# Aikku93/ulc-codec

Hardware: AMD Instinct MI355X
Metric: encode+decode Msamples/s at BlockSize=2048 stereo (channel-samples through encode+decode, VBR -50, 32 blocks per stream per call) (higher is better)
Workload: dtype f32; 1 GPU; vbr50 (configs[1] encode, configs[2] decode): Batch=4096 independent 44.1 kHz stereo streams/GPU x 32 blocks, BlockSize=2048, VBR -50; step = encode then decode; config=vbr50, mode=both, streams_per_gpu=4096, block_size=2048, channels=2, parallelism=batch split over 1 GPU(s), no collective on the data path

## Files before the change

### ulc-codec_amd/csrc/ulcx_enc.hip

```cpp
#include "ulcx_enc_dev.h"

static size_t ulcx_enc_xf_lds_bytes(int BS, int C) {
    if (BS > 8192) return (size_t)BS * 4;
    int ps = ulcx_xf_pad_shift(BS, C);
    size_t z = (size_t)4 * (BS + (BS >> ps)) * 4;
    size_t full = z + (size_t)BS * 2 + 32 + (C > 2 ? (size_t)BS * 2 : 0);
    return full <= ULCX_LDS_LIMIT ? full : z + (size_t)BS * 2 + 32;
}

static size_t ulcx_enc_xfa_lds_bytes(int BS, int C) {
    if (BS > 8192) return (size_t)BS * 4;
    int ps = ulcx_xf_pad_shift(BS, C);
    return (size_t)2 * (BS + (BS >> ps)) * 4 + (size_t)BS * 2 + 32;
}

#define CK(x) do { hipError_t e_ = (x); if (e_ != hipSuccess) { ulcx_set_error("%s: %s", #x, hipGetErrorString(e_)); return ULCX_ERR_HIP; } } while (0)
#define TRY(x) do { int rc_ = (x); if (rc_) return rc_; } while (0)

typedef void (*RangeKernel)(UlcxEncCtx, int, int);
typedef void (*PassKernel)(UlcxEncCtx, int);
typedef void (*CallKernel)(UlcxEncCtx);

static RangeKernel wc_energy_fn(const UlcxEncCtx &c) { return c.pcm16 ? k_wc_energy<int16_t> : k_wc_energy<float>; }
static RangeKernel wc_ef_fn(const UlcxEncCtx &c) { return c.pcm16 ? k_wc_ef<EF_NW, int16_t> : k_wc_ef<EF_NW, float>; }
static CallKernel state_update_fn(const UlcxEncCtx &c) { return c.pcm16 ? k_state_update<int16_t> : k_state_update<float>; }

template <typename IN> static RangeKernel xf_fn_in(const UlcxEncCtx &c, bool mdctOnly) {
    if (c.BS > 8192) return mdctOnly ? k_xfa_big<IN> : k_xf_big<IN>;
    if (c.C == 2) return mdctOnly ? k_xfa<true, IN> : k_xf<true, IN>;
    return mdctOnly ? k_xfa<false, IN> : k_xf<false, IN>;
}
static RangeKernel xf_fn(const UlcxEncCtx &c, bool mdctOnly) { return c.pcm16 ? xf_fn_in<int16_t>(c, mdctOnly) : xf_fn_in<float>(c, mdctOnly); }

template <int PASS> static PassKernel select_fn_pass(const UlcxEncCtx &c, bool pair, bool rates) {
#define SEL(R, L) (rates ? (PassKernel)k_select_wave_rates<R, L, PASS> : (PassKernel)k_select_wave<R, L, PASS>)
    switch (c.C * c.BS / 64) {
        case 128:
            if (pair) return rates ? k_select_pair_rates<64, 12, PASS> : k_select_pair<64, 12, PASS>;
            return SEL(128, 0);
        case 64: return c.lgBS == 11 ? SEL(64, 11) : SEL(64, 0);
        case 32: return SEL(32, 0);
        case 16: return SEL(16, 0);
        case 8:  return SEL(8, 0);
        case 4:  return SEL(4, 0);
        default: return nullptr;
    }
#undef SEL
}
static PassKernel select_fn(const UlcxEncCtx &c, bool pair, bool rates, int pass) {
    return pass == 1 ? select_fn_pass<1>(c, pair, rates) : pass == 2 ? select_fn_pass<2>(c, pair, rates) : select_fn_pass<0>(c, pair, rates);
}

static int allow_lds(const void *fn, size_t lds) {
    if (lds > 48 * 1024) CK(hipFuncSetAttribute(fn, hipFuncAttributeMaxDynamicSharedMemorySize, (int)lds));
    return ULCX_OK;
}

static void launch_wc_energy(const UlcxEncCtx &c, unsigned grid, hipStream_t st, int k0, int k1) {
    hipLaunchKernelGGL(wc_energy_fn(c), dim3(grid), dim3(WG), 0, st, c, k0, k1);
}

static void launch_wc_ef(const UlcxEncCtx &c, hipStream_t st, int k0, int k1) {
    static_assert(EF_LDS_BYTES <= 48 * 1024, "k_wc_ef: raise the dynamic LDS limit with hipFuncSetAttribute");
    hipLaunchKernelGGL(wc_ef_fn(c), dim3((c.B + EF_SPW - 1) / EF_SPW), dim3(EF_NW * 64), EF_LDS_BYTES, st, c, k0, k1);
}

static void launch_state_update(const UlcxEncCtx &c, hipStream_t st) {
    hipLaunchKernelGGL(state_update_fn(c), dim3(c.B), dim3(WG), 0, st, c);
}

const char *const ulcx_enc_stage_names[ULCX_ENC_STAGES_REPORTED] = {
    "k_wc_energy", "k_wc_forward", "k_wc_backward", "k_wc_integrate", "k_wc_decide",
    "k_xf", "k_cplx", "k_pbark", "k_mask",
    "k_select", "k_nbark", "(k_nline: gone)", "k_heapsel", "k_nsums", "k_tails", "k_encode_wave", "k_encode_units", "k_pack", "cbr_probe_passes", "k_state_update", "wc_pipeline_exposed",
};

struct StageMarks { hipEvent_t *ev; int stage; };
#define MARK(mk, s) do { if ((mk).ev) CK(hipEventRecord((mk).ev[(mk).stage++], s)); } while (0)

enum { ULCX_FRONT_ENCODE = 0, ULCX_FRONT_ANALYSE = 1, ULCX_FRONT_ANALYSE_KXF = 2, ULCX_FRONT_WC_ONLY = 3 };
static int launch_front(const UlcxEncCtx &c, hipStream_t st, StageMarks &mk, const UlcxEncAux &aux, const int what) {
    UlcxEncSync &sy = aux.sync;
    hipStream_t side = sy.side, side2 = sy.side2, side3 = sy.side3;
    const int SG = (c.B + 63) / 64;
    const int nCh = aux.wcPipe;
    const bool mdctOnly = (what == ULCX_FRONT_ANALYSE);
    const RangeKernel xf = (what == ULCX_FRONT_WC_ONLY) ? nullptr : xf_fn(c, mdctOnly);
    const size_t lds = mdctOnly ? ulcx_enc_xfa_lds_bytes(c.BS, c.C) : ulcx_enc_xf_lds_bytes(c.BS, c.C);
    if (xf) TRY(allow_lds((const void *)xf, lds));
    auto transform = [&](int k0, int k1) {
        if (xf) hipLaunchKernelGGL(xf, dim3((unsigned)((c.B * (k1 - k0) + 7) / 8) * 8), dim3(WG), lds, st, c, k0, k1);
    };
    const bool wcFuse = c.C == 2 && aux.wcFuse;
    aux.nXf = 0;
    if (nCh <= 1) {
        if (wcFuse) { MARK(mk, st); launch_wc_ef(c, st, 0, c.K);                                                  MARK(mk, st); }
        else {
        launch_wc_energy(c, (unsigned)(SG * ((c.K * c.BS) / 64)), st, 0, c.K);                                    MARK(mk, st);
        hipLaunchKernelGGL(k_wc_forward, dim3((c.B * 2 + 63) / 64), dim3(64), 0, st, c, 0, c.K);                  MARK(mk, st);
        }
        hipLaunchKernelGGL(k_wc_backward, dim3(SG * c.K), dim3(64), 0, st, c, 0, c.K);                            MARK(mk, st);
        hipLaunchKernelGGL(k_wc_integrate, dim3((c.B + 63) / 64), dim3(64), 0, st, c, 0, c.K);                    MARK(mk, st);
        hipLaunchKernelGGL(k_wc_decide, dim3((c.B * c.K + 63) / 64), dim3(64), 0, st, c, 0, c.K);                 MARK(mk, st);
        transform(0, c.K);
        MARK(mk, st);
        return ULCX_OK;
    }
    for (int i = 0; i < 5; i++) MARK(mk, st);
    const UlcxFrontPlan fp = ulcx_front_plan(c.K, nCh, aux.wcSteps);
    const int nW = fp.nW;
    const int *cut = fp.cut, *wcs = fp.wcs;
    CK(hipEventRecord(sy.wcStart, st));
    CK(hipStreamWaitEvent(side, sy.wcStart, 0));
    int jx = 0;
    for (int w = 0; w < nW; w++) {
        const int k0 = wcs[w], k1 = wcs[w + 1], kc = k1 - k0;
        if (wcFuse) launch_wc_ef(c, side, k0, k1);
        else {
            launch_wc_energy(c, (unsigned)(SG * ((kc * c.BS) / 64)), side, k0, k1);
            hipLaunchKernelGGL(k_wc_forward, dim3((c.B * 2 + 63) / 64), dim3(64), 0, side, c, k0, k1);
        }
        CK(hipEventRecord(sy.wcForward[w], side));
        CK(hipStreamWaitEvent(side2, sy.wcForward[w], 0));
        hipLaunchKernelGGL(k_wc_backward, dim3(SG * kc), dim3(64), 0, side2, c, k0, k1);
        CK(hipEventRecord(sy.wcBackward[w], side2));
        CK(hipStreamWaitEvent(side3, sy.wcBackward[w], 0));
        hipLaunchKernelGGL(k_wc_integrate, dim3((c.B + 63) / 64), dim3(64), 0, side3, c, k0, k1);
        hipLaunchKernelGGL(k_wc_decide, dim3((c.B * kc + 63) / 64), dim3(64), 0, side3, c, k0, k1);
        CK(hipEventRecord(sy.wcDecided[w], side3));
        while (jx < nCh && cut[jx + 1] <= k1) {
            CK(hipStreamWaitEvent(st, sy.wcDecided[w], 0));
            if (mk.ev) CK(hipEventRecord(sy.xfTiming[2 * jx], st));
            if (!(ULCX_DBG(c) & 0x2000))
            transform(cut[jx], cut[jx + 1]);
            if (mk.ev) CK(hipEventRecord(sy.xfTiming[2 * jx + 1], st));
            CK(hipEventRecord(sy.xfChunkDone[jx], st));
            jx++;
        }
    }
    aux.nXf = nCh;
    MARK(mk, st);
    for (int j = 0; j < nCh; j++) {
        CK(hipStreamWaitEvent(side, sy.xfChunkDone[j], 0));
        const int kc2 = cut[j + 1] - cut[j];
        if (what == ULCX_FRONT_ENCODE) hipLaunchKernelGGL(k_cplx, dim3((c.B * kc2 + 63) / 64), dim3(64), 0, side, c, cut[j], cut[j + 1]);
        else hipLaunchKernelGGL(k_cplxa, dim3((c.B * kc2 + 63) / 64), dim3(64), 0, side, c, cut[j], cut[j + 1]);
    }
    CK(hipEventRecord(sy.cplxChunksDone, side));
    return ULCX_OK;
}

struct EncPlan {
    int NB, N, nUnits;
    bool aside;
    int probes;
    size_t barkLds;
    bool selWave, selPair;
    size_t selLds;
    int ldsEntries, fbGrid; size_t heapLds;
    WaveCaps capS, capM, capF;
    bool haveFull, haveMid;
    int nsSlots;
};
static int enc_probes(const UlcxEncCtx &c, int N) {
    int n = 0;
    if (c.mode != ULCX_MODE_VBR || c.rates != nullptr) { n = 2; for (int m = N; m > 1; m >>= 1) n++; }
    return n;
}
static EncPlan enc_plan(const UlcxEncCtx &c, const UlcxEncAux &aux) {
    EncPlan p;
    p.NB = c.B * c.K; p.N = c.C * c.BS; p.nUnits = p.NB * c.C * 4;
    p.aside = aux.sync.side != nullptr;
    p.probes = enc_probes(c, p.N);
    p.barkLds = (size_t)c.barkRing * 3 * 64 * 8 + (size_t)2 * BK_TILE_FLOATS * 4;
    const int R = p.N / 64;
    p.selWave = (R == 4 || R == 8 || R == 16 || R == 32 || R == 64 || R == 128);
    p.selPair = (R == 128 && c.C == 2 && c.selPair);
    p.selLds = (size_t)(p.selPair ? 1 : 4) * ulcx_sel_lds_words(c.BS) * sizeof(float);
    p.ldsEntries = ((size_t)p.N * 8 <= ULCX_HEAP_LDS_BYTES) ? p.N : 0;
    p.heapLds = p.ldsEntries ? (size_t)p.N * 8 + (size_t)p.N / 8 : 0;
    p.fbGrid = p.NB < ULCX_HEAP_GRID ? p.NB : ULCX_HEAP_GRID;
    p.capS = { WAVE_SK, WAVE_SZ, WAVE_SN };
    p.capF = { (c.BS + 63) & ~63, ((c.BS / 2) + 63) & ~63, 4 * c.BS + 64 };
    while ((size_t)wavecaps_lds(p.capF) * 4 > 150 * 1024) {
        p.capF.k = (p.capF.k / 2 + 63) & ~63; p.capF.z = (p.capF.z / 2 + 63) & ~63; p.capF.nyb = p.capF.nyb / 2 + 32;
    }
    p.haveFull = p.capF.k > p.capS.k;
    p.capM = { 1024, 512, 4096 };
    p.haveMid = p.capM.k < p.capF.k;
    p.nsSlots = aux.nsSlots;
    return p;
}

static void launch_noise(const UlcxEncCtx &c, const EncPlan &p, hipStream_t s2) {
    if (c.barkRing) {
        hipLaunchKernelGGL(k_bark_uniform<true>, dim3((p.NB * c.C + 63) / 64), dim3(256), p.barkLds, s2, c);
        hipLaunchKernelGGL(k_bark_levels<true>, dim3((unsigned)(((size_t)p.NB * c.C * 32 + WG - 1) / WG)), dim3(WG), 0, s2, c);
    }
    hipLaunchKernelGGL(k_nbark, dim3((p.nUnits + 63) / 64), dim3(64), 0, s2, c, c.barkRing ? 1 : 0);
}

static int launch_psy(const UlcxEncCtx &c, const EncPlan &p, UlcxEncSync &sy, hipStream_t st, StageMarks &mk, bool cplxChunked) {
    if (c.barkRing) { TRY(allow_lds((const void *)k_bark_uniform<true>, p.barkLds)); TRY(allow_lds((const void *)k_bark_uniform<false>, p.barkLds)); }
    if (p.aside) {
        CK(hipEventRecord(sy.noiseFork, st));
        CK(hipStreamWaitEvent(sy.side3, sy.noiseFork, 0));
        if (cplxChunked) CK(hipStreamWaitEvent(sy.side3, sy.cplxChunksDone, 0));
        else hipLaunchKernelGGL(k_cplx, dim3((p.NB + 63) / 64), dim3(64), 0, sy.side3, c, 0, c.K);
        CK(hipEventRecord(sy.cplxDone, sy.side3));
        MARK(mk, st);
        launch_state_update(c, sy.side3);
        CK(hipEventRecord(sy.stateDone, sy.side3));
        CK(hipStreamWaitEvent(sy.side2, sy.noiseFork, 0));
        launch_noise(c, p, sy.side2);
        CK(hipEventRecord(sy.noiseDone, sy.side2));
    } else { hipLaunchKernelGGL(k_cplx, dim3((p.NB + 63) / 64), dim3(64), 0, st, c, 0, c.K);                MARK(mk, st); }
    const bool uniP = c.barkRing != 0;
    if (uniP) {
        hipLaunchKernelGGL(k_bark_uniform<false>, dim3((p.NB + 63) / 64), dim3(256), p.barkLds, st, c);
        hipLaunchKernelGGL(k_bark_levels<false>, dim3((unsigned)(((size_t)p.NB * 32 + WG - 1) / WG)), dim3(WG), 0, st, c);
    }
    hipLaunchKernelGGL(k_pbark, dim3((p.NB * 4 + 63) / 64), dim3(64), 0, st, c, uniP ? 1 : 0);            MARK(mk, st);
    MARK(mk, st);
    if (p.aside) CK(hipStreamWaitEvent(st, sy.cplxDone, 0));
    return ULCX_OK;
}

static int launch_select_wave(const UlcxEncCtx &c, const EncPlan &p, hipStream_t st, bool rates, int pass, int fin) {
    const PassKernel fn = select_fn(c, p.selPair, rates, pass);
    TRY(allow_lds((const void *)fn, p.selLds));
    if (p.selPair) hipLaunchKernelGGL(fn, dim3(p.NB), dim3(128), p.selLds, st, c, fin);
    else hipLaunchKernelGGL(fn, dim3((p.NB + 3) / 4), dim3(256), p.selLds, st, c, fin);
    return ULCX_OK;
}
static int launch_select(const UlcxEncCtx &c, const EncPlan &p, hipStream_t st, int fin) {
    if (!p.selWave) { hipLaunchKernelGGL(k_select, dim3(p.NB), dim3(WG), 0, st, c, fin); return ULCX_OK; }
    const bool rates = c.rates && c.selPass;
    TRY(launch_select_wave(c, p, st, rates, c.selPass, fin));
    if (rates && fin) TRY(launch_select_wave(c, p, st, true, 0, fin));
    return ULCX_OK;
}

static int launch_encode(const UlcxEncCtx &cc, const EncPlan &p, UlcxEncSync &sy, hipStream_t s2, int fin, StageMarks &mk) {
    const bool fb2 = (cc.fbMode == 2);
    const int NB = p.NB, fbW = NB < 128 ? NB : 128;
    if (cc.useGapSums) {
        const size_t glds = nsums_lds_bytes(p.N, cc.C);
        TRY(allow_lds((const void *)k_nsums, glds));
        const bool tailAside = !fb2 && p.aside;
        const unsigned tg = (unsigned)((p.nUnits + TAILS_U - 1) / TAILS_U);
        if (tailAside) {
            CK(hipEventRecord(sy.tailFork, s2));
            CK(hipStreamWaitEvent(sy.side2, sy.tailFork, 0));
            hipLaunchKernelGGL(k_tails, dim3(tg), dim3(WG), 0, sy.side2, cc, fin);
            CK(hipEventRecord(sy.tailDone, sy.side2));
        }
        const int nsGrid = NB < p.nsSlots ? NB : p.nsSlots;
        hipLaunchKernelGGL(k_nsums, dim3(fb2 ? fbW : nsGrid), dim3(WG), glds, s2, cc, fin);
        MARK(mk, s2);
        if (tailAside) CK(hipStreamWaitEvent(s2, sy.tailDone, 0));
        else hipLaunchKernelGGL(k_tails, dim3(fb2 ? fbW : tg), dim3(WG), 0, s2, cc, fin);
        MARK(mk, s2);
    } else { MARK(mk, s2); MARK(mk, s2); }
    if (cc.useWave) {
        const int nBC = NB * cc.C;
        hipLaunchKernelGGL(k_encode_wave<true>, dim3(fb2 ? fbW : (nBC + 3) / 4), dim3(256), (size_t)wavecaps_lds(p.capS) * 4 + 16, s2, cc, fin, p.capS, p.haveFull ? 0 : 2);
        if (p.haveFull) {
            const WaveCaps capR = (p.haveMid && (fb2 || (p.probes > 0 && !fin))) ? p.capM : p.capF;
            hipLaunchKernelGGL(k_encode_wave<false>, dim3(fb2 ? fbW : ((nBC + 3) / 4 < 512 ? (nBC + 3) / 4 : 512)), dim3(256), (size_t)wavecaps_lds(capR) * 4 + 16, s2, cc, fin, capR, 1);
        }
    }
    MARK(mk, s2);
    hipLaunchKernelGGL(k_encode_units, dim3(fb2 ? fbW : (p.nUnits + 63) / 64), dim3(64), 0, s2, cc, fin);
    MARK(mk, s2);
    if (!fin && !fb2) hipLaunchKernelGGL(k_rate_step, dim3((NB + 255) / 256), dim3(256), 0, s2, cc);
    else hipLaunchKernelGGL(k_pack, dim3(fb2 ? (fbW + 3) / 4 : (NB + 3) / 4), dim3(256), 0, s2, cc, fin);
    MARK(mk, s2);
    return ULCX_OK;
}

static UlcxEncCtx exact_ctx(const UlcxEncCtx &c, int lo) { UlcxEncCtx cf = c; cf.fbMode = 2; cf.fbLo = lo; cf.fbHi = lo + c.rankSlots; return cf; }
static void exact_sort(const UlcxEncCtx &c, const EncPlan &p, hipStream_t s2, int lo) {
    const UlcxEncCtx cf = exact_ctx(c, lo);
    if (p.ldsEntries) hipLaunchKernelGGL(k_heapsel_pipe, dim3(p.fbGrid), dim3(64), p.heapLds, s2, cf, p.probes > 0 ? 1 : 0);
    else hipLaunchKernelGGL(k_heapsel, dim3(p.fbGrid), dim3(64), p.heapLds, s2, cf, p.ldsEntries);
}
static int exact_passes(const UlcxEncCtx &c, const EncPlan &p, UlcxEncSync &sy, hipStream_t s2, int lo) {
    const UlcxEncCtx cf = exact_ctx(c, lo);
    StageMarks none = { nullptr, 0 };
    for (int pass = 0; pass <= p.probes; pass++) {
        const int fin = (pass == p.probes) ? 1 : 0;
        const bool fromSort = (p.probes == 0 && p.ldsEntries);
        if (!fromSort) hipLaunchKernelGGL(k_keep_ranks, dim3(p.fbGrid), dim3(WG), 0, s2, cf, fin);
        if (cf.useWave && !(fromSort && lo == 0)) CK(hipMemsetAsync(cf.slow + p.NB + 1, 0, sizeof(int), s2));
        TRY(launch_encode(cf, p, sy, s2, fin, none));
    }
    return ULCX_OK;
}

static int launch_passes(UlcxEncCtx &c, const EncPlan &p, UlcxEncSync &sy, hipStream_t st, StageMarks &mk, bool first) {
    const int NB = p.NB;
    StageMarks none = { nullptr, 0 };
    for (int pass = 0; pass <= p.probes; pass++) {
        const int fin = (pass == p.probes) ? 1 : 0;
        StageMarks &m = (pass == 0) ? mk : none;
        const bool async_fb = p.aside && fin;
        if (c.useWave && pass > 0) CK(hipMemsetAsync(c.slow, 0, sizeof(int) * ((size_t)NB + 2), st));
        c.selPass = (p.probes > 0 && !c.keyFinal) ? (pass == 0 ? 1 : 2) : 0;
        TRY(launch_select(c, p, st, fin));
        MARK(m, st);
        if (async_fb) {
            CK(hipEventRecord(sy.exactFork, st));
            CK(hipStreamWaitEvent(sy.side, sy.exactFork, 0));
            exact_sort(c, p, sy.side, 0);
        }
        if (pass == 0) {
            if (first) {
                if (p.aside) CK(hipStreamWaitEvent(st, sy.noiseDone, 0));
                else launch_noise(c, p, st);
            }
            MARK(m, st); MARK(m, st);
        }
        if (async_fb) {
            CK(hipEventRecord(sy.exactFork2, st));
            CK(hipStreamWaitEvent(sy.side, sy.exactFork2, 0));
            TRY(exact_passes(c, p, sy, sy.side, 0));
            for (int lo = c.rankSlots; lo < NB; lo += c.rankSlots) {
                exact_sort(c, p, sy.side, lo);
                TRY(exact_passes(c, p, sy, sy.side, lo));
            }
            CK(hipEventRecord(sy.exactJoin, sy.side));
        }
        MARK(m, st);
        UlcxEncCtx cm = c; cm.fbMode = 1;
        TRY(launch_encode(cm, p, sy, st, fin, m));
        if (async_fb) CK(hipStreamWaitEvent(st, sy.exactJoin, 0));
    }
    if (!p.aside) {
        for (int lo = 0; lo < NB; lo += c.rankSlots) {
            exact_sort(c, p, st, lo);
            TRY(exact_passes(c, p, sy, st, lo));
        }
    }
    return ULCX_OK;
}

int ulcx_enc_launch_ladder(const UlcxEncCtx *rungs, int nRungs, hipStream_t st, hipEvent_t *ev, const UlcxEncAux &aux) {
    UlcxEncCtx c = rungs[0];
    UlcxEncSync &sy = aux.sync;
    const EncPlan p = enc_plan(c, aux);
    StageMarks mk = { ev, 0 }, none = { nullptr, 0 };
    if (p.probes) CK(hipMemsetAsync(c.cbrLive, 0, sizeof(int), st));
    if (c.barkRing) CK(hipMemsetAsync(c.decCount, 0, sizeof(int), st));
    if (nRungs > 1) CK(hipMemsetAsync(c.fbCount + 1, 0, sizeof(int), st));
    MARK(mk, st);
    TRY(launch_front(c, st, mk, aux, ULCX_FRONT_ENCODE));
    if (ULCX_DBG(c) & 0x6000) { MARK(mk, st); return ULCX_OK; }
    TRY(launch_psy(c, p, sy, st, mk, aux.wcPipe > 1));
    if (!p.selWave) { ulcx_enc_finalize_keys(c, st); c.keyFinal = 1; }
    TRY(allow_lds((const void *)k_heapsel, p.heapLds)); TRY(allow_lds((const void *)k_heapsel_pipe, p.heapLds));
    if (p.haveFull && (size_t)wavecaps_lds(p.capF) * 4 > 48 * 1024) CK(hipFuncSetAttribute((const void *)k_encode_wave<false>, hipFuncAttributeMaxDynamicSharedMemorySize, wavecaps_lds(p.capF) * 4 + 16));
    TRY(launch_passes(c, p, sy, st, mk, true));
    for (int r = 1; r < nRungs; r++) {
        UlcxEncCtx cr = rungs[r];
        cr.keyFinal = c.keyFinal;
        EncPlan pr = p;
        pr.probes = enc_probes(cr, p.N);
        if (pr.probes) CK(hipMemsetAsync(cr.cbrLive, 0, sizeof(int), st));
        ulcx_enc_rung_arm(cr, st);
        TRY(launch_passes(cr, pr, sy, st, none, false));
    }
    MARK(mk, st);
    if (p.aside) CK(hipStreamWaitEvent(st, sy.stateDone, 0));
    else launch_state_update(c, st);
    MARK(mk, st);
    CK(hipGetLastError());
    return ULCX_OK;
}

int ulcx_enc_launch(const UlcxEncCtx &c, hipStream_t st, hipEvent_t *ev, const UlcxEncAux &aux) {
    return ulcx_enc_launch_ladder(&c, 1, st, ev, aux);
}

int ulcx_analyse_launch(const UlcxEncCtx &c, hipStream_t st, hipEvent_t *ev, const UlcxEncAux &aux, int useKxf) {
    const int what = !c.cplxOut ? ULCX_FRONT_WC_ONLY : useKxf ? ULCX_FRONT_ANALYSE_KXF : ULCX_FRONT_ANALYSE;
    if (what == ULCX_FRONT_ANALYSE_KXF && c.barkRing) CK(hipMemsetAsync(c.decCount, 0, sizeof(int), st));
    StageMarks mk = { ev, 0 };
    MARK(mk, st);
    TRY(launch_front(c, st, mk, aux, what));
    if (aux.wcPipe > 1) CK(hipStreamWaitEvent(st, aux.sync.cplxChunksDone, 0));
    else hipLaunchKernelGGL(k_cplxa, dim3((c.B * c.K + 63) / 64), dim3(64), 0, st, c, 0, c.K);
    MARK(mk, st);
    while (mk.ev && mk.stage < ULCX_ENC_STAGES) MARK(mk, st);
    launch_state_update(c, st);
    MARK(mk, st);
    CK(hipGetLastError());
    return ULCX_OK;
}
```

### ulc-codec_amd/csrc/ulcx_enc_wr.hip

```cpp
#include "ulcx_enc_dev.h"

__device__ __forceinline__ float run_amplitude(const float *pairs, int start, int n) {
    const float2 *d = (const float2 *)(pairs + (start / 2) * 2);
    const int np = (n + (start & 1) + 1) / 2;
    float sum = 0.0f, sumw = 0.0f;
    int q = 0;
    for (; q + 8 <= np; q += 8) {
        float2 p[8];
#pragma unroll
        for (int u = 0; u < 8; u++) p[u] = d[q + u];
#pragma unroll
        for (int u = 0; u < 8; u++) { sum += p[u].y; sumw += p[u].x; }
    }
    for (; q < np; q++) { float2 p = d[q]; sum += p.y; sumw += p.x; }
    return (sum == 0.0f) ? -1.0f : ulcx_expf(sum / sumw);
}

#define NS_KW 2

#define NS_BK 7

struct NsPre { uint32_t kw[NS_KW]; float bk[NS_BK]; int wc; };

__device__ __forceinline__ void nsums_fetch(const UlcxEncCtx &c, int blk, NsPre &p) {
// ... 547 lines not shown
                uint32_t b = (lane >= s) ? lv : 0u;
#define STEP(ctl, rmask) { uint32_t o = (uint32_t)__builtin_amdgcn_update_dpp((int)0xFFFFFFFFu, (int)a, ctl, rmask, 0xf, false); a = o < a ? o : a; \
                           uint32_t q = (uint32_t)__builtin_amdgcn_update_dpp(0, (int)b, ctl, rmask, 0xf, false); b = q > b ? q : b; }
                ULCX_DPP_STEPS(STEP)
#undef STEP
                if (open) { a = cmn < a ? cmn : a; b = cmx > b ? cmx : b; }
                const bool brk = (__uint_as_float(b) > __uint_as_float(a) * 4.0f) && (open || lane > s);
                const unsigned long long m = __ballot(brk);
                if (m == 0ull) {
                    if (lane >= s) myz = nZ;
                    cmn = (uint32_t)__builtin_amdgcn_readlane((int)a, 63); cmx = (uint32_t)__builtin_amdgcn_readlane((int)b, 63);
                    open = true;
                    break;
                }
                const int t = __builtin_ctzll(m);
                if (lane >= s && lane < t) myz = nZ;
                const uint32_t zm = t > 0 ? (uint32_t)__builtin_amdgcn_readlane((int)b, t - 1) : cmx;
                if (lane == 0 && nZ < E2_ZCAP) ((uint32_t *)zmax)[nZ] = zm;
                nZ++;
                s = t; open = false;
                if (base + t >= nK) break;
            }
            if (i < nK) kz[i] = (uint16_t)myz;
        }
        if (open) { if (lane == 0 && nZ < E2_ZCAP) ((uint32_t *)zmax)[nZ] = cmx; nZ++; }
        WAVE_SYNC();
        if (nZ <= E2_ZCAP && __builtin_amdgcn_readfirstlane((int)((uint32_t *)zmax)[nZ - 1]) == 0) nZ--;
        if (nZ > E2_ZCAP) overflow = true;
    }
    WAVE_SYNC();
    if ((ULCX_DBG(c) >> 8) == 2) { if (lane == 0) c.unitNyb[gid] = 0; return; }

    if (!overflow) {
        int run = 0;
        for (int base = 0; base < nZ; base += 64) {
            int z = base + lane;
            int qn = 0;
            if (z < nZ) { int qi = build_quantizer(zmax[z]); zqi[z] = (int8_t)qi; }
            WAVE_SYNC();
            if (z < nZ) {
                int qi = zqi[z];
                int prev = (z > 0) ? zqi[z - 1] : -1;
                if (qi != prev) qn = ((z > 0) ? 1 : 0) + ((qi - 5 < 0xE) ? 1 : 2);
            }
            int tot, ex = wave_excl_scan(qn, lane, tot);
            if (z < nZ) zpre[z] = run + ex + qn;
            run += tot;
        }
    }
    WAVE_SYNC();
    if ((ULCX_DBG(c) >> 8) == 3) { if (lane == 0) c.unitNyb[gid] = 0; return; }

    int nC = 0;
    if (!overflow) {
        bool prevCodedCarry = true;
        for (int base = 0; base < nK; base += 64) {
            int kk = base + lane;
            bool coded = false; int qn = 0, idx = 0, z = 0;
            if (kk < nK) {
                z = kz[kk]; idx = kidx[kk];
                float cq = kval[kk] * (float)(1u << zqi[z]);
                coded = !(fabsf(cq) < 2.5f);
                qn = quant_coef(cq, 7);
            }
            unsigned long long m = __ballot(coded);
            unsigned long long valid = __ballot(kk < nK);
            bool prevCoded = (lane == 0) ? prevCodedCarry : (((m >> (lane - 1)) & 1) != 0);
            int pos = nC + __popcll(m & ((1ull << lane) - 1));
            if (coded) { kidx[pos] = (uint16_t)(idx | (prevCoded ? 0x8000 : 0)); kz[pos] = (uint16_t)z; ((int *)kval)[pos] = qn; }
            int lastValid = 63 - __clzll(valid);
            prevCodedCarry = ((m >> lastValid) & 1) != 0;
            nC += __popcll(m);
        }
    }
    WAVE_SYNC();
    if ((ULCX_DBG(c) >> 8) == 4) { if (lane == 0) c.unitNyb[gid] = 0; return; }

    int total = 0;
    if (!overflow) {
        auto gap_amps = [&](int m) {
            float2 a = make_float2(-2.0f, -2.0f);
            if (m < nC) {
                const int raw = kidx[m], idx = raw & 0x7FFF, start = (m > 0) ? (kidx[m - 1] & 0x7FFF) + 1 : 0;
                if (idx - start >= 16 && (raw & 0x8000) && c.useGapSums) a = gapU[idx];
            }
            return a;
        };
        float2 ampR = gap_amps(lane);
        for (int base = 0; base < nC; base += 64) {
            int m = base + lane;
            unsigned long long lo = 0, hi = 0; int cnt = 0, pre = 0, z = 0, zp = -1, qn = 0;
            const float2 ampN = gap_amps(m + 64);
            if (m < nC) {
                int raw = kidx[m];
                int idx = raw & 0x7FFF;
                int start = (m > 0) ? (kidx[m - 1] & 0x7FFF) + 1 : 0;
                z = kz[m]; zp = (m > 0) ? kz[m - 1] : -1;
                qn = ((int *)kval)[m];
                pre = zpre[z] - ((zp >= 0) ? zpre[zp] : 0);
                int zr = idx - start;
                const float amp0 = ampR.x, amp1 = ampR.y;
                gap_codes(start, zr, (float)(1u << zqi[z]), coefU, src, ubase, amp0, amp1, amp0 > -1.5f ? gapU + idx : nullptr, lo, hi, cnt, (ULCX_DBG(c) & 0x40) != 0);
            }
            int mine = (m < nC) ? pre + cnt + 1 : 0;
            int tot, ex = wave_excl_scan(mine, lane, tot);
            if (cnt > 32) overflow = true;
            int p = total + ex;
            if (m < nC && finalPass && p + mine <= E2_NYBCAP && cnt <= 32) {
                for (int zz = zp + 1; zz <= z; zz++) {
                    int qi = zqi[zz], prev = (zz > 0) ? zqi[zz - 1] : -1;
                    if (qi != prev) {
                        if (zz > 0) nyb[p++] = 0xF;
                        int sft = qi - 5;
                        if (sft < 0xE) nyb[p++] = (uint8_t)sft; else { nyb[p++] = 0xE; nyb[p++] = (uint8_t)(sft - 0xE); }
                    }
                }
                for (int q = 0; q < cnt; q++) nyb[p++] = (uint8_t)(((q < 16) ? (lo >> (4 * q)) : (hi >> (4 * (q - 16)))) & 0xF);
                nyb[p++] = (uint8_t)(qn & 0xF);
            }
            total += tot;
            ampR = ampN;
        }
        overflow = __any(overflow);
    }
    if ((ULCX_DBG(c) >> 8) == 5) { if (lane == 0) c.unitNyb[gid] = 0; return; }

    if (!overflow) {
        int zlast = (nC > 0) ? kz[nC - 1] : -1;
        int nextCoded = (nC > 0) ? (kidx[nC - 1] & 0x7FFF) + 1 : 0;
        int n = S - nextCoded;
        int prevQ = (nZ > 0) ? zqi[nZ - 1] : -1;
        int qtail = ((nZ > 0) ? zpre[nZ - 1] : 0) - ((zlast >= 0) ? zpre[zlast] : 0);
        int nq = 0, nd = 0;
        if (n > 4 && prevQ != -1 && n >= 16) {
            float sx, sx2, sxy, sy, sw;
            if (c.useGapSums && __float_as_int(tsB.y) == ubase + nextCoded) {
                sx = tsA.x; sx2 = tsA.y; sxy = tsA.z; sy = tsA.w; sw = tsB.x;
            } else {
                const int p0 = (ubase + nextCoded) / 2;
                int np = (n + (nextCoded & 1) + 1) / 2;
                float acc = 0.0f;
                if (lane < 5) {
                    for (int i = 0; i < np; i++) {
                        float2 pv = pair_demand(src, p0 + i);
                        float x = i * 2.0f;
                        float wx = pv.x * x;
                        float term = (lane == 0) ? wx : (lane == 1) ? wx * x : (lane == 2) ? x * pv.y : (lane == 3) ? pv.y : pv.x;
                        acc += term;
                    }
                }
                sx = __shfl(acc, 0); sx2 = __shfl(acc, 1); sxy = __shfl(acc, 2); sy = __shfl(acc, 3); sw = __shfl(acc, 4);
            }
            hfext_from_sums(sx, sx2, sxy, sy, sw, (float)(1u << prevQ), nq, nd);
        }
        int tailN = 0;
        if (n > 4) tailN = ((prevQ != -1) ? 1 : 0) + (nq ? 4 : 2);
        else if (n > 0) tailN = 2;
        int p = total + qtail;
        if (finalPass && lane == 0 && p + tailN <= E2_NYBCAP) {
            int q0 = total;
            for (int zz = zlast + 1; zz < nZ; zz++) {
                int qi = zqi[zz], prev = (zz > 0) ? zqi[zz - 1] : -1;
                if (qi != prev) {
                    if (zz > 0) nyb[q0++] = 0xF;
                    int sft = qi - 5;
                    if (sft < 0xE) nyb[q0++] = (uint8_t)sft; else { nyb[q0++] = 0xE; nyb[q0++] = (uint8_t)(sft - 0xE); }
                }
            }
            if (n > 4) {
                if (prevQ != -1) nyb[p++] = 0xF;
                if (nq) { nyb[p++] = 0xF; nyb[p++] = (uint8_t)(nq - 1); nyb[p++] = (uint8_t)((nd >> 4) & 0xF); nyb[p++] = (uint8_t)(nd & 0xF); }
                else { nyb[p++] = 0xE; nyb[p++] = 0xF; }
            } else if (n > 0) { nyb[p++] = 0x0; nyb[p++] = (uint8_t)(n - 1); }
        }
        total += qtail + tailN;
        if (total > E2_NYBCAP) overflow = true;
    }
    const bool direct = xch != nullptr;
    if (overflow) {
        if (direct && ch == 0 && lane == 0) __hip_atomic_store(xch, XCH_WORD(0, 0, 1, seq), __ATOMIC_RELAXED, __HIP_MEMORY_SCOPE_WORKGROUP);
        if (lane == 0) {
            int old = atomicOr(&c.slow[blk], failBit);
            if (failBit == 1 && !(old & 1)) {
                const int NBq = c.B * c.K, which = (c.fbMode == 2) ? 1 : 0;
                int q = atomicAdd(&c.slow[NBq + which], 1);
                c.slow[NBq + 2 + which * NBq + q] = blk;
            }
        }
        return;
    }
    WAVE_SYNC();
    if (lane == 0) c.unitNyb[gid] = total;
    if (!finalPass) return;
    if (direct) {
        int o = 1; uint32_t prevNyb = (uint32_t)wc & 0xFu;
        bool ok = true;
        if (ch == 0) {
            if (lane == 0) __hip_atomic_store(xch, XCH_WORD(total, total ? nyb[total - 1] : prevNyb, 0, seq), __ATOMIC_RELAXED, __HIP_MEMORY_SCOPE_WORKGROUP);
        } else {
            unsigned long long v64;
            for (;;) {
                v64 = __hip_atomic_load(xch, __ATOMIC_RELAXED, __HIP_MEMORY_SCOPE_WORKGROUP);
                if ((uint32_t)(v64 >> 32) == (uint32_t)seq) break;
                __builtin_amdgcn_s_sleep(2);
            }
            const uint32_t v = (uint32_t)__builtin_amdgcn_readfirstlane((int)(uint32_t)v64);
            ok = !((v >> 20) & 1u);
            o = 1 + (int)(v & 0xFFFFu); prevNyb = (v >> 16) & 0xFu;
        }
        if (ok) {
            const int end = o + total;
            const int bEnd = ch == 0 ? end >> 1 : (end + 1) >> 1;
            uint8_t *outB = c.out + (size_t)blk * c.slot;
            for (int b = (o >> 1) + lane; b < bEnd; b += 64) {
                const int q0 = 2 * b - o;
                const unsigned lo4 = q0 >= 0 ? nyb[q0] : prevNyb;
                const unsigned hi4 = q0 + 1 < total ? nyb[q0 + 1] : 0u;
                if (b < c.slot) outB[b] = (uint8_t)(lo4 | (hi4 << 4));
            }
            if (ch == 1 && lane == 0) { c.bits[blk] = (end * 4 + 7) & ~7; atomicOr(&c.slow[blk], 4); }
            return;
        }
    }
    uint8_t *dst = c.unitBuf + (size_t)blk * c.C * c.unitCap + (size_t)ch * c.unitCap + 2 * off + 8 * j;
    int nb = (total + 1) / 2;
    for (int b = lane; b < nb; b += 64) {
        unsigned lo4 = nyb[2 * b];
        unsigned hi4 = (2 * b + 1 < total) ? nyb[2 * b + 1] : 0;
        dst[b] = (uint8_t)(lo4 | (hi4 << 4));
    }
}

template <bool SMALL>
__global__ __launch_bounds__(256, SMALL ? EW_LB : 1) void k_encode_wave(UlcxEncCtx c, int finalPass, WaveCaps caps, int phase) {
    if (probes_over(c, finalPass)) return;
    extern __shared__ float e2all[];
    const int wv = __builtin_amdgcn_readfirstlane(threadIdx.x >> 6), lane = threadIdx.x & 63;
    const WaveCaps capS = { WAVE_SK, WAVE_SZ, WAVE_SN };
    const int ldsPerWave = SMALL ? wavecaps_lds(capS) : wavecaps_lds(caps);
    float *e2 = (float *)((char *)e2all + (size_t)wv * ldsPerWave);
    const int NBq = c.B * c.K, which = (c.fbMode == 2) ? 1 : 0;
    const int *queue = c.slow + NBq + 2 + which * NBq;
    int nBlk = (phase == 1) ? c.slow[NBq + which] : (c.fbMode == 2) ? fb_count(c) : NBq;
    unsigned long long *xchAll = (unsigned long long *)((char *)e2all + 4 * (size_t)ldsPerWave);
    const bool directOK = finalPass && c.C == 2 && phase != 1 && c.directPack && (long long)gridDim.x * 4 >= (long long)nBlk * c.C;
    if (directOK) { if (threadIdx.x < 2) xchAll[threadIdx.x] = 0; __syncthreads(); }
    int seq = 0;
    for (int u = blockIdx.x * 4 + wv; u < nBlk * c.C; u += gridDim.x * 4) {
        seq++;
        int blk = u / c.C, ch = u - blk * c.C;
        if (phase == 1) blk = queue[blk];
        else {
            if (c.fbMode == 2) blk = c.fbList[c.fbLo + blk];
            if (skip_block(c, blk, finalPass)) continue;
        }
        int s = blk / c.K, k = blk % c.K;
        const int nW0 = c.BS >> 5;
        const uint32_t kwPre = (lane < nW0) ? c.keep[(size_t)blk * (c.C * c.BS / 32) + (size_t)ch * nW0 + lane] : 0u;
        int wc = c.wcArr[(size_t)s * (c.maxK + 2) + k + 1];
        const bool whole = (c.BS >> (ulcx_pattern(wc) & 7)) == c.BS;
        for (int j = 0; j < 4; j++) {
            encode_unit_wave<SMALL>(c, finalPass, blk, ch, j, wc, lane, e2, caps, phase ? 2 : 1, (directOK && whole && j == 0) ? xchAll + (wv >> 1) : nullptr, seq, kwPre, j == 0);
            WAVE_SYNC();
        }
    }
}

__device__ void pack_block(const UlcxEncCtx &c, int finalPass, int blk) {
    int lane = threadIdx.x & 63;
    if (skip_block(c, blk, finalPass)) return;
    if (finalPass && c.useWave && (c.slow[blk] & 4)) return;
    int s = blk / c.K, k = blk % c.K;
    int wc = c.wcArr[(size_t)s * (c.maxK + 2) + k + 1];
    int nU = c.C * 4;
    const int *un = c.unitNyb + (size_t)blk * nU;
    int hdr = (wc & 8) ? 2 : 1;
    int total = hdr;
    for (int u = 0; u < nU; u++) total += un[u];
    int bitsTot = ((total * 4) + 7) & ~7;
    if (!finalPass) {
        if (lane == 0) {
            int budget = c.cbrBudget[blk];
            int lo = c.cbrLo[blk], hi = c.cbrHi[blk], nOut = c.nout[blk];
            bool stop = false;
            if (bitsTot < budget) lo = nOut;
            else if (bitsTot > budget) hi = nOut - 1;
            else { lo = nOut; stop = true; }
            if (stop || !(lo < hi - 1)) { c.cbrDone[blk] = 1; c.nout[blk] = lo; if (c.fbMode != 2) atomicSub(c.cbrLive, 1); }
            else c.nout[blk] = (int)((unsigned)(lo + hi) / 2u);
            c.cbrLo[blk] = lo; c.cbrHi[blk] = hi;
            if (c.selPass && c.fbMode != 2 && nOut > 0) {
                const uint32_t T = c.selT[blk];
                uint4 w = c.selWin[blk];
                if (bitsTot > budget) { w.x = T; w.z = (uint32_t)nOut; }
                else { w.y = T; w.w = (uint32_t)nOut; }
                c.selWin[blk] = w;
            }
        }
        return;
    }
    uint8_t *out = c.out + (size_t)blk * c.slot;
    int nBytes = bitsTot / 8;
    const uint8_t *ub = c.unitBuf + (size_t)blk * c.C * c.unitCap;
    for (int b = lane; b < nBytes; b += 64) {
        unsigned byte = 0;
        for (int h = 0; h < 2; h++) {
            int q = 2 * b + h;
            unsigned nyb = 0;
            if (q < hdr) nyb = (q == 0) ? (wc & 0xF) : ((wc >> 4) & 0xF);
            else if (q < total) {
                int r = q - hdr;
                int u = 0;
                while (r >= un[u]) { r -= un[u]; u++; }
                int ch = u >> 2, j = u & 3;
                int d, off, S;
                unit_geom(wc, j, c.BS, d, off, S);
                const uint8_t *src = ub + (size_t)ch * c.unitCap + 2 * off + 8 * j;
                nyb = (src[r >> 1] >> ((r & 1) * 4)) & 0xF;
            }
            byte |= nyb << (4 * h);
        }
        if (b < c.slot) out[b] = (uint8_t)byte;
    }
    if (lane == 0) c.bits[blk] = bitsTot;
}

__global__ __launch_bounds__(256) void k_rate_step(UlcxEncCtx c) {
    if (probes_over(c, 0)) return;
    const int blk = blockIdx.x * 256 + threadIdx.x;
    bool ended = false;
    if (blk < c.B * c.K && !skip_block(c, blk, 0)) {
        const int s = blk / c.K, k = blk % c.K;
        const int wc = c.wcArr[(size_t)s * (c.maxK + 2) + k + 1];
        const int nU = c.C * 4;
        const int *un = c.unitNyb + (size_t)blk * nU;
        int total = (wc & 8) ? 2 : 1;
        for (int u = 0; u < nU; u++) total += un[u];
        const int bitsTot = ((total * 4) + 7) & ~7;
        const int budget = c.cbrBudget[blk];
        int lo = c.cbrLo[blk], hi = c.cbrHi[blk];
        const int nOut = c.nout[blk];
        bool stop = false;
        if (bitsTot < budget) lo = nOut;
        else if (bitsTot > budget) hi = nOut - 1;
        else { lo = nOut; stop = true; }
        if (stop || !(lo < hi - 1)) { c.cbrDone[blk] = 1; c.nout[blk] = lo; ended = true; }
        else c.nout[blk] = (int)((unsigned)(lo + hi) / 2u);
        c.cbrLo[blk] = lo; c.cbrHi[blk] = hi;
        if (c.selPass && nOut > 0) {
            const uint32_t T = c.selT[blk];
            uint4 w = c.selWin[blk];
            if (bitsTot > budget) { w.x = T; w.z = (uint32_t)nOut; }
            else { w.y = T; w.w = (uint32_t)nOut; }
            c.selWin[blk] = w;
        }
    }
    const unsigned long long e = __ballot(ended);
    if (e && (threadIdx.x & 63) == 0) atomicSub(c.cbrLive, (int)__popcll(e));
}

__global__ __launch_bounds__(256) void k_pack(UlcxEncCtx c, int finalPass) {
    if (probes_over(c, finalPass)) return;
    const int wv = threadIdx.x >> 6;
    if (c.fbMode != 2) { const int blk = blockIdx.x * 4 + wv; if (blk < c.B * c.K) pack_block(c, finalPass, blk); return; }
    int n = fb_count(c);
    for (int v = blockIdx.x * 4 + wv; v < n; v += gridDim.x * 4) pack_block(c, finalPass, c.fbList[c.fbLo + v]);
}

int ulcx_enc_nsums_slots(int BS, int C) {
    const size_t lds = nsums_lds_bytes(C * BS, C);
    if (lds > 48 * 1024 && hipFuncSetAttribute((const void *)k_nsums, hipFuncAttributeMaxDynamicSharedMemorySize, (int)lds) != hipSuccess) { (void)hipGetLastError(); return 0; }
    int dev = 0, cus = 0, per = 0;
    if (hipGetDevice(&dev) != hipSuccess || hipDeviceGetAttribute(&cus, hipDeviceAttributeMultiprocessorCount, dev) != hipSuccess) { (void)hipGetLastError(); return 0; }
    if (hipOccupancyMaxActiveBlocksPerMultiprocessor(&per, (const void *)k_nsums, WG, lds) != hipSuccess) { (void)hipGetLastError(); return 0; }
    return cus * per;
}

template __global__ void k_encode_wave<false>(UlcxEncCtx, int, WaveCaps, int);
template __global__ void k_encode_wave<true>(UlcxEncCtx, int, WaveCaps, int);
```

Measured before the change: 56370 Msamples/s.

## Overlap pbark on side stream and vectorize nybble packing with wave scan

Moves the k_pbark launch onto the side3 stream, ahead of the wait on the chunked cplx work, when bark-ring and chunked cplx are active, so it overlaps with the main-stream bark kernels. Rewrites the final bitstream packing for blocks with at most 64 units. A wave-wide exclusive scan now builds per-unit start offsets in shared memory, and each lane emits a 32-bit word, using a funnel shift for the aligned-in-unit case. This replaces per-nybble linear unit searches and byte stores. The cost is added shared memory and an extra wave sync, plus the risk of a race if pbark's inputs on the side stream depend on work still running on the main stream.

Result: no change. 56480 Msamples/s, median of 6 (+0.2%).

```diff
diff --git a/ulc-codec_amd/csrc/ulcx_enc.hip b/ulc-codec_amd/csrc/ulcx_enc.hip
--- a/ulc-codec_amd/csrc/ulcx_enc.hip
+++ b/ulc-codec_amd/csrc/ulcx_enc.hip
@@ -202,9 +202,13 @@
 
 static int launch_psy(const UlcxEncCtx &c, const EncPlan &p, UlcxEncSync &sy, hipStream_t st, StageMarks &mk, bool cplxChunked) {
     if (c.barkRing) { TRY(allow_lds((const void *)k_bark_uniform<true>, p.barkLds)); TRY(allow_lds((const void *)k_bark_uniform<false>, p.barkLds)); }
+    const bool uniP = c.barkRing != 0;
+    const bool pbAside = p.aside && uniP && cplxChunked;
+    const dim3 pbGrid((p.NB * 4 + 63) / 64);
     if (p.aside) {
         CK(hipEventRecord(sy.noiseFork, st));
         CK(hipStreamWaitEvent(sy.side3, sy.noiseFork, 0));
+        if (pbAside) hipLaunchKernelGGL(k_pbark, pbGrid, dim3(64), 0, sy.side3, c, 1);
         if (cplxChunked) CK(hipStreamWaitEvent(sy.side3, sy.cplxChunksDone, 0));
         else hipLaunchKernelGGL(k_cplx, dim3((p.NB + 63) / 64), dim3(64), 0, sy.side3, c, 0, c.K);
         CK(hipEventRecord(sy.cplxDone, sy.side3));
@@ -215,12 +219,12 @@
         launch_noise(c, p, sy.side2);
         CK(hipEventRecord(sy.noiseDone, sy.side2));
     } else { hipLaunchKernelGGL(k_cplx, dim3((p.NB + 63) / 64), dim3(64), 0, st, c, 0, c.K);                MARK(mk, st); }
-    const bool uniP = c.barkRing != 0;
     if (uniP) {
         hipLaunchKernelGGL(k_bark_uniform<false>, dim3((p.NB + 63) / 64), dim3(256), p.barkLds, st, c);
         hipLaunchKernelGGL(k_bark_levels<false>, dim3((unsigned)(((size_t)p.NB * 32 + WG - 1) / WG)), dim3(WG), 0, st, c);
     }
-    hipLaunchKernelGGL(k_pbark, dim3((p.NB * 4 + 63) / 64), dim3(64), 0, st, c, uniP ? 1 : 0);            MARK(mk, st);
+    if (!pbAside) hipLaunchKernelGGL(k_pbark, pbGrid, dim3(64), 0, st, c, uniP ? 1 : 0);
+    MARK(mk, st);
     MARK(mk, st);
     if (p.aside) CK(hipStreamWaitEvent(st, sy.cplxDone, 0));
     return ULCX_OK;
diff --git a/ulc-codec_amd/csrc/ulcx_enc_wr.hip b/ulc-codec_amd/csrc/ulcx_enc_wr.hip
--- a/ulc-codec_amd/csrc/ulcx_enc_wr.hip
+++ b/ulc-codec_amd/csrc/ulcx_enc_wr.hip
@@ -873,27 +873,73 @@
     uint8_t *out = c.out + (size_t)blk * c.slot;
     int nBytes = bitsTot / 8;
     const uint8_t *ub = c.unitBuf + (size_t)blk * c.C * c.unitCap;
-    for (int b = lane; b < nBytes; b += 64) {
-        unsigned byte = 0;
-        for (int h = 0; h < 2; h++) {
-            int q = 2 * b + h;
-            unsigned nyb = 0;
-            if (q < hdr) nyb = (q == 0) ? (wc & 0xF) : ((wc >> 4) & 0xF);
-            else if (q < total) {
-                int r = q - hdr;
-                int u = 0;
-                while (r >= un[u]) { r -= un[u]; u++; }
-                int ch = u >> 2, j = u & 3;
-                int d, off, S;
-                unit_geom(wc, j, c.BS, d, off, S);
-                const uint8_t *src = ub + (size_t)ch * c.unitCap + 2 * off + 8 * j;
-                nyb = (src[r >> 1] >> ((r & 1) * 4)) & 0xF;
-            }
-            byte |= nyb << (4 * h);
-        }
-        if (b < c.slot) out[b] = (uint8_t)byte;
+    if (nU > 64) {
+        for (int b = lane; b < nBytes; b += 64) {
+            unsigned byte = 0;
+            for (int h = 0; h < 2; h++) {
+                int q = 2 * b + h;
+                unsigned nyb = 0;
+                if (q < hdr) nyb = (q == 0) ? (wc & 0xF) : ((wc >> 4) & 0xF);
+                else if (q < total) {
+                    int r = q - hdr;
+                    int u = 0;
+                    while (r >= un[u]) { r -= un[u]; u++; }
+                    int ch = u >> 2, j = u & 3;
+                    int d, off, S;
+                    unit_geom(wc, j, c.BS, d, off, S);
+                    const uint8_t *src = ub + (size_t)ch * c.unitCap + 2 * off + 8 * j;
+                    nyb = (src[r >> 1] >> ((r & 1) * 4)) & 0xF;
+                }
+                byte |= nyb << (4 * h);
+            }
+            if (b < c.slot) out[b] = (uint8_t)byte;
+        }
+        if (lane == 0) c.bits[blk] = bitsTot;
+        return;
+    }
+    __shared__ int pkStart[4][65], pkSrc[4][64];
+    int *uStart = pkStart[threadIdx.x >> 6], *uSrc = pkSrc[threadIdx.x >> 6];
+    {
+        const int sz = lane < nU ? un[lane] : 0;
+        int tot, ex = wave_excl_scan(sz, lane, tot);
+        int d, off = 0, S;
+        if (lane < nU) unit_geom(wc, lane & 3, c.BS, d, off, S);
+        uStart[lane] = hdr + ex;
+        uSrc[lane] = (lane >> 2) * c.unitCap + 2 * off + 8 * (lane & 3);
+        if (lane == 0) uStart[64] = hdr + tot;
+    }
+    WAVE_SYNC();
+    if (nBytes > c.slot) nBytes = c.slot;
+    const bool wordOut = ((uintptr_t)out & 3) == 0;
+    for (int w = lane; w < (nBytes + 3) >> 2; w += 64) {
+        const int q0 = 8 * w;
+        int u = -1;
+        for (int i = 0; i < nU; i++) u += (uStart[i] <= q0) ? 1 : 0;
+        uint32_t val = 0;
+        if (u >= 0 && q0 + 8 <= uStart[u + 1]) {
+            const int r = q0 - uStart[u], sh = (r & 7) * 4;
+            const uint32_t *src = (const uint32_t *)(ub + uSrc[u]) + (r >> 3);
+            const uint32_t a = src[0], b = sh ? src[1] : 0u;
+            val = __funnelshift_r(a, b, sh);
+        } else {
+            for (int i = 0; i < 8; i++) {
+                const int q = q0 + i;
+                unsigned nyb = 0;
+                if (q < hdr) nyb = (q == 0) ? (wc & 0xF) : ((wc >> 4) & 0xF);
+                else if (q < total) {
+                    while (u < 0 || q >= uStart[u + 1]) u++;
+                    const int r = q - uStart[u];
+                    nyb = (ub[uSrc[u] + (r >> 1)] >> ((r & 1) * 4)) & 0xF;
+                }
+                val |= nyb << (4 * i);
+            }
+        }
+        const int b0 = 4 * w;
+        if (wordOut && b0 + 4 <= nBytes) *(uint32_t *)(out + b0) = val;
+        else for (int i = 0; i < 4 && b0 + i < nBytes; i++) out[b0 + i] = (uint8_t)(val >> (8 * i));
     }
     if (lane == 0) c.bits[blk] = bitsTot;
+    WAVE_SYNC();
 }
 
 __global__ __launch_bounds__(256) void k_rate_step(UlcxEncCtx c) {
```
